# danieldugas/DeepMimic_mujoco

Hardware: AMD Instinct MI355X
Metric: env-steps/sec (whole node), 34-DoF humanoid, 4096 envs, at 1/2/4/8 MI355X (higher is better)
Workload: dtype f32

## Files before the change

### deepmimic_mujoco_amd/csrc/dm_abi.hip

```cpp
#include "../../include/deepmimic_hip.h"
#include "dm_device.h"
#include "dm_topology.h"

#include <math.h>
#include <stdio.h>
#include <string.h>

#include <string>
#include <vector>

#include "dm_kernels.hip"

struct DmEngine {
  DmConfig cfg;
  DmModel model;
  int N = 0;
  DmDev *dT = nullptr;
  float *dState = nullptr;
  float *dArScratch = nullptr;
  float *dClipRows[DM_MAX_CLIPS] = {nullptr};
  float *dClipReset[DM_MAX_CLIPS] = {nullptr};
  int clipL[DM_MAX_CLIPS] = {0};
  int clipFlags[DM_MAX_CLIPS] = {0};
  float *debug = nullptr;
// ... 85 lines not shown
    T.b_chainb[b] = cb;
  }
  for (int k = 0; k < DM_NV; k++) {
    int j = m.dof_jnt[k];
    T.d_body[k] = m.dof_body[k];
    T.d_act[k] = -1;
    T.d_limited[k] = (m.jnt_type[j] == DM_JNT_HINGE) ? m.jnt_limited[j] : 0;
    for (int i = 0; i < 3; i++) T.d_axis[k][i] = (float)m.jnt_axis[j][i];
    T.d_arm[k] = (float)m.dof_armature[k]; T.d_damp[k] = (float)m.dof_damping[k];
    T.d_invw[k] = (float)m.dof_invweight0[k];
    T.d_lo[k] = (float)m.jnt_range[j][0]; T.d_hi[k] = (float)m.jnt_range[j][1];
    int n = 0;
    for (int a = m.dof_parent[k]; a >= 0 && n < DMK_MAXANC; a = m.dof_parent[a]) T.d_anc[k][n++] = (uint8_t)a;
    T.d_nanc[k] = n;
    for (int d = 0; d < n; d++) T.d_ancabs[k][d] = T.d_anc[k][n - 1 - d];
    T.d_pbody[k] = m.body_parent[m.dof_body[k]];
  }
  for (int k = 0; k < DM_NV; k++) {
    for (int a = 0; a < T.d_nanc[k]; a++) T.d_desc[T.d_anc[k][a]] |= 1ull << k;
    T.nanc_pack[k >> 4] |= (uint64_t)T.d_nanc[k] << (4 * (k & 15));
    for (int a = 0; a < T.d_nanc[k]; a++) T.d_ancm[k] |= 1ull << T.d_anc[k][a];
    T.d_madr[k] = m.dof_Madr[k];
  }
  for (int a = 0; a < DM_NU; a++) {
    int k = m.act_dof[a];
    T.d_act[k] = a; T.d_gear[k] = (float)m.act_gear[a];
    T.d_clo[k] = (float)m.act_ctrlrange[a][0]; T.d_chi[k] = (float)m.act_ctrlrange[a][1];
  }
  for (int g = 0; g < DM_NGEOM; g++) {
    T.g_body[g] = m.geom_body[g]; T.g_type[g] = m.geom_type[g]; T.g_condim[g] = m.geom_condim[g];
    for (int i = 0; i < 3; i++) { T.g_pos[g][i] = (float)m.geom_pos[g][i]; T.g_size[g][i] = (float)m.geom_size[g][i]; }
    const double *q = m.geom_quat[g];
    double w = q[0], x = q[1], y = q[2], z = q[3];
    double M[9] = {w * w + x * x - y * y - z * z, 2 * (x * y - w * z), 2 * (x * z + w * y),
                   2 * (x * y + w * z), w * w - x * x + y * y - z * z, 2 * (y * z - w * x),
                   2 * (x * z - w * y), 2 * (y * z + w * x), w * w - x * x - y * y + z * z};
    for (int i = 0; i < 9; i++) T.g_mat[g][i] = (float)M[i];
    T.g_rbound[g] = (float)m.geom_rbound[g]; T.g_margin[g] = (float)m.geom_margin[g];
    T.g_mu[g] = (float)m.geom_friction[g][0];
  }
  for (int p = 0; p < DM_MAXPAIR; p++) { T.p_g1[p] = (int16_t)m.pair_geom1[p]; T.p_g2[p] = (int16_t)m.pair_geom2[p]; }
  for (int p = 0; p < m.npair; p++) {
    int g1 = m.pair_geom1[p], g2 = m.pair_geom2[p];
    DmPairDev &pr = T.pairs[p];
    pr.g1 = (int16_t)g1; pr.g2 = (int16_t)g2;
    pr.t1 = (int8_t)m.geom_type[g1]; pr.t2 = (int8_t)m.geom_type[g2];
    pr.margin = (float)fmax(m.geom_margin[g1], m.geom_margin[g2]);
    pr.rbsum = (float)((m.geom_type[g1] == DM_GEOM_PLANE ? 0.0 : m.geom_rbound[g1]) + m.geom_rbound[g2]);
    for (int i = 0; i < 3; i++) { pr.z1[i] = (float)m.geom_size[g1][i]; pr.z2[i] = (float)m.geom_size[g2][i]; }
  }
  int p = 0;
  for (int b = 0; b < DMK_MAXANC; b++)
    for (int a = 0; a <= b; a++) { T.tri_a[p] = (uint8_t)a; T.tri_b[p] = (uint8_t)b; p++; }
}

static int check_model(DmEngine *e, const DmModel &m) {
  if (m.nq != DM_NQ || m.nv != DM_NV || m.nu != DM_NU || m.nbody != DM_NBODY || m.ngeom != DM_NGEOM)
    return fail(e, DM_EINVAL, "model dimensions do not match the compiled-in humanoid3d dimensions");
  if (m.integrator != DM_INT_RK4 && m.integrator != DM_INT_EULER) return fail(e, DM_EINVAL, "integrator must be RK4 or Euler");
  if (m.npair < 0 || m.npair > DM_MAXPAIR) return fail(e, DM_EINVAL, "npair out of range");
  for (int b = 1; b < DM_NBODY; b++) {
    if (m.body_quat[b][0] != 1.0) return fail(e, DM_EINVAL, "kernels assume identity body quaternions");
    if (m.body_dofnum[b] != 1 && m.body_dofnum[b] != 3 && m.body_dofnum[b] != 6)
      return fail(e, DM_EINVAL, "kernels assume 1- or 3-hinge bodies under a free root");
    if (m.body_depth[b] < 1 || m.body_depth[b] > 4) return fail(e, DM_EINVAL, "tree depth > 4");
  }
  for (int j = 0; j < DM_NJNT; j++)
    for (int i = 0; i < 3; i++)
      if (m.jnt_pos[j][i] != 0.0) return fail(e, DM_EINVAL, "kernels assume joint anchors at the body origin");
  if (m.jnt_type[0] != DM_JNT_FREE || m.jnt_body[0] != 1) return fail(e, DM_EINVAL, "joint 0 must be the free root");
  for (int k = 0; k < DM_NV; k++)
    if (m.dof_parent[k] != topo::PARENT[k] || m.dof_Madr[k] != topo::MADR[k])
      return fail(e, DM_EINVAL, "dof tree differs from the compiled-in topology (regenerate csrc/dm_topology.h)");
  for (int b = 0; b < DM_NBODY; b++)
    if (m.body_parent[b] != topo::BPARENT[b])
      return fail(e, DM_EINVAL, "body tree differs from the compiled-in topology (regenerate csrc/dm_topology.h)");
  return DM_OK;
}

extern "C" int dm_create(const DmModel *model, const DmConfig *cfg, DmHandle *out) {
  if (!model || !cfg || !out || cfg->num_envs < 1) return DM_EINVAL;
  int ndev = 0;
  if (hipGetDeviceCount(&ndev) != hipSuccess || ndev <= 0) return DM_ENODEV;
  DmEngine *e = new DmEngine();
  e->cfg = *cfg;
  e->model = *model;
  e->N = cfg->num_envs;
  if (const char *w = getenv("DM_WAVES")) e->waves = atoi(w);
  int rc = check_model(e, *model);
  if (rc != DM_OK) { fprintf(stderr, "dm_create: %s\n", e->err.c_str()); delete e; return rc; }
  if (hipSetDevice(cfg->device) != hipSuccess) { delete e; return DM_ENODEV; }
  DmDev T;
  build_tables(*model, T);
  if (hipMalloc(&e->dT, sizeof(DmDev)) != hipSuccess) { delete e; return DM_ENOMEM; }
  hipMemcpy(e->dT, &T, sizeof(DmDev), hipMemcpyHostToDevice);
  size_t sb = (size_t)e->N * DMK_STATE_STRIDE * sizeof(float);
  if (hipMalloc(&e->dState, sb) != hipSuccess) { hipFree(e->dT); delete e; return DM_ENOMEM; }
  std::vector<float> init((size_t)e->N * DMK_STATE_STRIDE, 0.f);
  for (int i = 0; i < e->N; i++)
    for (int k = 0; k < DM_NQ; k++) init[(size_t)i * DMK_STATE_STRIDE + DMS_QPOS + k] = (float)model->qpos0[k];
  hipMemcpy(e->dState, init.data(), sb, hipMemcpyHostToDevice);
  if (hipMalloc(&e->dArScratch, (size_t)e->N * DMK_MAXROW * DMK_MAXROW * sizeof(float)) != hipSuccess) {
    hipFree(e->dState); hipFree(e->dT); delete e; return DM_ENOMEM;
  }
  if (hipMalloc(&e->dOrder, e->N * sizeof(int32_t)) != hipSuccess || hipMalloc(&e->dCost, e->N * sizeof(int32_t)) != hipSuccess) {
    hipFree(e->dArScratch); hipFree(e->dState); hipFree(e->dT); delete e; return DM_ENOMEM;
// ... 352 lines not shown
```

### deepmimic_mujoco_amd/csrc/dm_device.h

```cpp
#pragma once

#include <hip/hip_runtime.h>
#include <stdint.h>

#include "../../include/dm_model.h"

#define DMK_NQ DM_NQ
#define DMK_NV DM_NV
#define DMK_NU DM_NU
#define DMK_NB DM_NBODY
#define DMK_NG DM_NGEOM
#define DMK_MAXCON DM_MAXCON
#define DMK_MAXROW DM_MAXROW
#define DMK_LANEROW 64
#define DMK_REGROW 32
#define DMK_MSTRIDE 35
#define DMK_MAXANC 12
#define DMK_STATE_STRIDE 144
#define DMK_CLIP_ROW 80

struct DmPairDev {
  int16_t g1, g2;
  int8_t t1, t2, pad0, pad1;
  float margin, rbsum;
  float z1[3], z2[3];
};

struct DmDev {
  float timestep, tolerance, pgs_scale, gravity[3];
  float K, B;
  float solimp[5];
  float total_mass_inv;
  float qpos0[36];
  int32_t iterations, npair;
  int32_t torso_body, rfoot_geom, lfoot_geom, floor_geom;
  int32_t ee_geom[4];
  int32_t b_parent[16], b_depth[16], b_dofadr[16], b_dofnum[16];
  float b_pos[16][3], b_ipos[16][3], b_inertia[16][6], b_mass[16], b_invw[16];
  uint32_t b_subtree[16];
  uint64_t b_chain[16];
  uint32_t b_chainb[16];
  int32_t d_body[DM_NV], d_nanc[DM_NV], d_act[DM_NV], d_limited[DM_NV];
  float d_axis[DM_NV][3];
  float d_arm[DM_NV], d_damp[DM_NV], d_invw[DM_NV], d_lo[DM_NV], d_hi[DM_NV];
  float d_gear[DM_NV], d_clo[DM_NV], d_chi[DM_NV];
  uint8_t d_anc[DM_NV][DMK_MAXANC];
  uint8_t d_ancabs[DM_NV][DMK_MAXANC + 4];
  uint64_t d_desc[DM_NV];
  int32_t d_pbody[DM_NV];
  uint64_t nanc_pack[3];
  uint64_t d_ancm[DM_NV];
  int32_t d_madr[DM_NV];
  int32_t g_body[16], g_type[16], g_condim[16];
  float g_pos[16][3], g_mat[16][9], g_size[16][3], g_rbound[16], g_margin[16], g_mu[16];
  int16_t p_g1[DM_MAXPAIR], p_g2[DM_MAXPAIR];
  DmPairDev pairs[DM_MAXPAIR];
  uint8_t tri_a[80], tri_b[80];
};

struct EnvLds {
  float qpos[36], qvel[36], warm[36], ctrl[28];
  float qacc_smooth[36], qacc[36];
  float cs[36][2];
  float xpos[DMK_NB][3], xquat[DMK_NB][4], xmat[DMK_NB][9], xipos[DMK_NB][3];
  float xaxis[DMK_NV][3];
  float gpos[DMK_NG][3], gmat[DMK_NG][9];
  float com[4];
  float cinert[DMK_NB][10];
  float cdof[DMK_NV][8];
  float cvel[DMK_NB][6];
  float M[DM_NM + 2];
  float dinv[36], dsqrtinv[36];
  float rk[5][36], rkq[4];
  float c_dist[DMK_MAXCON], c_pos[DMK_MAXCON][3], c_frame[DMK_MAXCON][9];
  int32_t c_g1[DMK_MAXCON], c_g2[DMK_MAXCON];
#ifdef DM_PROFILE
  unsigned long long prof_t, prof_t0; unsigned prof[16], prof_stage[4];
#endif
  int32_t info[8];
  int16_t rowinfo[DMK_MAXROW];
  union {
    struct {
      float crb[DMK_NB][10];
      float qloc[DMK_NB][8];
      union {
        struct { float cdofdot[DMK_NV][6]; float cacc[DMK_NB][6]; };
        alignas(16) float mbuf[DMK_NV][8];
      };
      float cfrc[DMK_NB][6], cfrcsub[DMK_NB][6];
    } v;
    struct {
      float tr[20][DM_NV + 1];
    } fin;
    struct {
      float poly[2][16][3];
      float cand[8][8];
      int32_t ncand;
    } bb;
  } u;
};

#define DMS_QPOS 0
#define DMS_QVEL 35
#define DMS_WARM 69
#define DMS_CTRL 103
#define DMS_IDX 131
#define DMS_EPLEN 132
#define DMS_EPREW 133
#define DMS_CLIP 134
#define DMS_RCNT 135
#define DMS_F8R 136
// ... 39 lines not shown
```

### deepmimic_mujoco_amd/csrc/dm_kernels.hip

```cpp
#include "../../include/deepmimic_hip.h"
#include "dm_device.h"
#include "dm_rng.h"
#include "dm_topology.h"

#include <math.h>

#include <type_traits>

#define SYNC()                                              \
  do {                                                      \
    __builtin_amdgcn_fence(__ATOMIC_RELEASE, "wavefront");  \
    __builtin_amdgcn_wave_barrier();                        \
    __builtin_amdgcn_fence(__ATOMIC_ACQUIRE, "wavefront");  \
  } while (0)
#define DMK_ENVS_PER_BLOCK 1
#ifndef DMK_WAVES_PER_SIMD
#define DMK_WAVES_PER_SIMD 2
#endif
#ifdef DM_PROFILE
#define PROF_DECL do { if ((threadIdx.x & 63) == 0) { for (int _i = 0; _i < 16; _i++) g_S.prof[_i] = 0; for (int _i = 0; _i < 4; _i++) g_S.prof_stage[_i] = 0; g_S.prof_t = g_S.prof_t0 = __builtin_amdgcn_s_memtime(); } } while (0)
#define PROF_STAGE(i) do { if ((threadIdx.x & 63) == 0 && (i) < 4) g_S.prof_stage[i] = (unsigned)(__builtin_amdgcn_s_memtime() - g_S.prof_t0); } while (0)
#define PROF(i) do { if ((threadIdx.x & 63) == 0) { unsigned long long _t = __builtin_amdgcn_s_memtime(); g_S.prof[i] += (unsigned)(_t - g_S.prof_t); g_S.prof_t = _t; } } while (0)
#if DM_PROFILE == 2
#define PROF2(i) PROF(i)
#else
#define PROF2(i) do {} while (0)
#endif
#else
#define PROF2(i) do {} while (0)
#define PROF_STAGE(i) do {} while (0)
#define PROF_DECL do {} while (0)
#define PROF(i) do {} while (0)
#endif
typedef __attribute__((address_space(3))) const float *lds_cfloat_p;
typedef float lds_f2v __attribute__((ext_vector_type(2)));
typedef float lds_f4v __attribute__((ext_vector_type(4)));
typedef float mfma_f16v __attribute__((ext_vector_type(16)));
#ifndef DMK_MFMA_MIN_ROWS
#define DMK_MFMA_MIN_ROWS 8
#endif
typedef const __attribute__((address_space(1))) DmDev GDev;
typedef const __attribute__((address_space(1))) DmPairDev GPair;
#define MINVALF 1e-15f
#define MAXVALF 1e10f

namespace {

template <int I, int N>
struct StaticFor {
  template <class F>
  static __device__ __forceinline__ void run(F &&f) {
    if constexpr (I < N) {
      if (f(std::integral_constant<int, I>{})) StaticFor<I + 1, N>::run(f);
    }
  }
};

__device__ __forceinline__ float rl(float v, int lane) {
  return __int_as_float(__builtin_amdgcn_readlane(__float_as_int(v), lane));
}
template <unsigned long long MASK>
__device__ __forceinline__ float lane_sel(float a, float b) {
  float out;
  asm("v_cndmask_b32_e64 %0, %1, %2, %3" : "=v"(out) : "v"(b), "v"(a), "s"(MASK));
  return out;
}
template <unsigned long long MASK>
__device__ __forceinline__ int lane_sel_i(int a, int b) {
  int out;
  asm("v_cndmask_b32_e64 %0, %1, %2, %3" : "=v"(out) : "v"(b), "v"(a), "s"(MASK));
  return out;
}
template <int N>
__device__ __forceinline__ void sgpr_batch(float (&a)[topo::FS_SLOTS]) {
  static_assert(N >= 1 && N <= 8 && topo::FS_SLOTS == 8, "one asm statement per batch size");
  if constexpr (N == 1) asm("" : "+s"(a[0]));
  if constexpr (N == 2) asm("" : "+s"(a[0]), "+s"(a[1]));
  if constexpr (N == 3) asm("" : "+s"(a[0]), "+s"(a[1]), "+s"(a[2]));
  if constexpr (N == 4) asm("" : "+s"(a[0]), "+s"(a[1]), "+s"(a[2]), "+s"(a[3]));
  if constexpr (N == 5) asm("" : "+s"(a[0]), "+s"(a[1]), "+s"(a[2]), "+s"(a[3]), "+s"(a[4]));
  if constexpr (N == 6) asm("" : "+s"(a[0]), "+s"(a[1]), "+s"(a[2]), "+s"(a[3]), "+s"(a[4]), "+s"(a[5]));
  if constexpr (N == 7) asm("" : "+s"(a[0]), "+s"(a[1]), "+s"(a[2]), "+s"(a[3]), "+s"(a[4]), "+s"(a[5]), "+s"(a[6]));
  if constexpr (N == 8) asm("" : "+s"(a[0]), "+s"(a[1]), "+s"(a[2]), "+s"(a[3]), "+s"(a[4]), "+s"(a[5]), "+s"(a[6]), "+s"(a[7]));
}
__device__ __forceinline__ void factor_columns(float (&C)[DMK_NV]) {
  float d[topo::FS_SLOTS], m[topo::FS_SLOTS], rk[DMK_NV], Cs[DMK_NV];
  StaticFor<0, topo::FS_NOPS>::run([&](auto nc) {
    constexpr topo::FactorOp o = topo::FACTOR_SCHED[decltype(nc)::value];
    if constexpr (o.op == topo::FS_DIAG) d[o.slot] = rl(C[o.k], o.k);
    if constexpr (o.op == topo::FS_RCP) rk[o.k] = __builtin_amdgcn_rcpf(d[o.slot]);
    if constexpr (o.op == topo::FS_SCALE) Cs[o.k] = C[o.k] * rk[o.k];
    if constexpr (o.op == topo::FS_BCAST) m[o.slot] = rl(Cs[o.k], o.i);
    if constexpr (o.op == topo::FS_FMA) C[o.i] = fmaf(-m[o.slot], C[o.k], C[o.i]);
    if constexpr (o.op == topo::FS_FENCE) sgpr_batch<o.slot>(m);
    if constexpr (o.op == topo::FS_DFENCE) sgpr_batch<o.slot>(d);
// ... 375 lines not shown
  S.u.bb.ncand = cnt;
}

__device__ __noinline__ float impedance_pow(float x, float mid, float power) {
  return (x <= mid) ? powf(x, power) / powf(mid, power - 1) : 1 - powf(1 - x, power) / powf(1 - mid, power - 1);
}
__device__ __forceinline__ float impedance(const float *solimp, float pos, float margin) {
  float dmin = solimp[0], dmax = solimp[1], width = solimp[2], mid = solimp[3], power = solimp[4];
  if (dmin == dmax || width <= MINVALF) return 0.5f * (dmin + dmax);
  float x = fabsf(pos - margin) / width;
  if (x >= 1) return dmax;
  if (x <= 0) return dmin;
  float y;
  if (power == 1) y = x;
  else if (power == 2) y = (x <= mid) ? x * x / mid : 1 - (1 - x) * (1 - x) / (1 - mid);
  else y = impedance_pow(x, mid, power);
  return dmin + y * (dmax - dmin);
}

}

__shared__ EnvLds g_S;

#define bp (T.b_parent[lb])
#define bdofadr (T.b_dofadr[lb])
#define bdofnum (T.b_dofnum[lb])
#define bpos (T.b_pos[lb])
#define bipos (T.b_ipos[lb])
#define binert (T.b_inertia[lb])
#define bsub (T.b_subtree[lb])
#define baxis(j) (T.d_axis[(bdofadr + (j)) < DMK_NV ? (bdofadr + (j)) : 0])
#define dbody (T.d_body[lk])
#define dnanc (T.d_nanc[lk])
#define dact (T.d_act[lk])
#define dlimited (T.d_limited[lk])
#define darm (T.d_arm[lk])
#define ddamp (T.d_damp[lk])
#define dlo (T.d_lo[lk])
#define dhi (T.d_hi[lk])
#define dgear (T.d_gear[lk])
#define dclo (T.d_clo[lk])
#define dchi (T.d_chi[lk])
#define gbody (T.g_body[lg])
#define gposl (T.g_pos[lg])
#define gmatl (T.g_mat[lg])

template <bool DAMP2 = false>
__device__ __forceinline__ float fwd_smooth(GDev &T, const int lane, const float rhs = 0.f) {
  EnvLds &S = g_S;
  const int lb = lane < DMK_NB ? lane : 0;
  const int lk = lane < DMK_NV ? lane : 0;
  const int lg = lane < DMK_NG ? lane : 0;
  const bool isbody = lane >= 1 && lane < DMK_NB, isdof = lane < DMK_NV;
  const float bmass = (lane < DMK_NB) ? T.b_mass[lb] : 0.f;
  const int b_dofadr = T.b_dofadr[lb], b_dofnum = T.b_dofnum[lb];
  const uint32_t b_chain4 = T.b_chainb[lb];
  const unsigned b_sub = T.b_subtree[lb];
  const int d_body = T.d_body[lk], d_nanc = T.d_nanc[lk], d_pbody = T.d_pbody[lk];
  const float mtot_inv = T.total_mass_inv;

  if constexpr (!DAMP2) {
  {
    float q[4] = {S.qpos[3], S.qpos[4], S.qpos[5], S.qpos[6]};
    quat_normalize(q);
    SYNC();
    if (lane < 4) S.qpos[3 + lane] = (lane == 0) ? q[0] : (lane == 1) ? q[1] : (lane == 2) ? q[2] : q[3];
    if (lane >= 6 && lane < DMK_NV) {
      float sn, cs;
      sincosf(0.5f * S.qpos[lane + 1], &sn, &cs);
      S.cs[lane][0] = cs; S.cs[lane][1] = sn;
    }
    SYNC();
  }
  PROF2(12);
  if (isbody) {
    float q[4] = {1.f, 0.f, 0.f, 0.f};
    if (lb == 1) {
      for (int i = 0; i < 4; i++) q[i] = S.qpos[3 + i];
    } else {
      {
        const int k = b_dofadr;
        const float al[3] = {T.d_axis[k][0], T.d_axis[k][1], T.d_axis[k][2]};
        S.xaxis[k][0] = al[0]; S.xaxis[k][1] = al[1]; S.xaxis[k][2] = al[2];
        const float c = S.cs[k][0], sn = S.cs[k][1];
        q[0] = c; q[1] = al[0] * sn; q[2] = al[1] * sn; q[3] = al[2] * sn;
      }
#pragma unroll
      for (int j = 1; j < 3; j++) {
        if (j < b_dofnum) {
          const int k = b_dofadr + j;
          const float al[3] = {T.d_axis[k][0], T.d_axis[k][1], T.d_axis[k][2]};
          float ax[3], ql[4], qn[4];
          quat_rot(ax, q, al);
          S.xaxis[k][0] = ax[0]; S.xaxis[k][1] = ax[1]; S.xaxis[k][2] = ax[2];
          const float c = S.cs[k][0], sn = S.cs[k][1];
          ql[0] = c; ql[1] = al[0] * sn; ql[2] = al[1] * sn; ql[3] = al[2] * sn;
          quat_mul(qn, q, ql);
          q[0] = qn[0]; q[1] = qn[1]; q[2] = qn[2]; q[3] = qn[3];
        }
      }
    }
    for (int i = 0; i < 4; i++) S.u.v.qloc[lb][i] = q[i];
    for (int i = 0; i < 3; i++) S.u.v.qloc[lb][4 + i] = (lb == 1) ? S.qpos[i] : T.b_pos[lb][i];
  }
  SYNC();
  if (isbody) {
    float q[4], pos[3];
    for (int i = 0; i < 4; i++) q[i] = S.u.v.qloc[1][i];
    for (int i = 0; i < 3; i++) pos[i] = S.u.v.qloc[1][4 + i];
#pragma unroll
    for (int c = 1; c < 4; c++) {
      const int cb = (b_chain4 >> (8 * c)) & 0xFF;
      if (cb != 0) {
        float ql[4], pl[3], t[3], qn[4];
        for (int i = 0; i < 4; i++) ql[i] = S.u.v.qloc[cb][i];
        for (int i = 0; i < 3; i++) pl[i] = S.u.v.qloc[cb][4 + i];
        quat_rot(t, q, pl);
        pos[0] += t[0]; pos[1] += t[1]; pos[2] += t[2];
        quat_mul(qn, q, ql);
        q[0] = qn[0]; q[1] = qn[1]; q[2] = qn[2]; q[3] = qn[3];
      }
    }
    quat_normalize(q);
    float m9[9], tv[3];
    quat2mat(m9, q);
    const float ip[3] = {T.b_ipos[lb][0], T.b_ipos[lb][1], T.b_ipos[lb][2]};
    mat_vec(tv, m9, ip);
    for (int i = 0; i < 3; i++) { S.xpos[lb][i] = pos[i]; S.xipos[lb][i] = pos[i] + tv[i]; }
    for (int i = 0; i < 4; i++) S.xquat[lb][i] = q[i];
    for (int i = 0; i < 9; i++) S.xmat[lb][i] = m9[i];
  }
  SYNC();
  PROF2(13);
  float com[3];
  {
    float ax[3] = {0.f, 0.f, 0.f};
    if (lane >= 6 && isdof) {
      const float pq[4] = {S.xquat[d_pbody][0], S.xquat[d_pbody][1], S.xquat[d_pbody][2], S.xquat[d_pbody][3]};
      const float al[3] = {S.xaxis[lk][0], S.xaxis[lk][1], S.xaxis[lk][2]};
      quat_rot(ax, pq, al);
    } else if (lane >= 3 && lane < 6) {
      ax[0] = S.xmat[1][lane - 3]; ax[1] = S.xmat[1][3 + lane - 3]; ax[2] = S.xmat[1][6 + lane - 3];
    }
    if (lane < DMK_NG) {
      const int gb = T.g_body[lg];
      float bm[9], tv[3], gl[3] = {T.g_pos[lg][0], T.g_pos[lg][1], T.g_pos[lg][2]}, gm[9];
      for (int i = 0; i < 9; i++) { bm[i] = S.xmat[gb][i]; gm[i] = T.g_mat[lg][i]; }
      mat_vec(tv, bm, gl);
      for (int i = 0; i < 3; i++) S.gpos[lg][i] = S.xpos[gb][i] + tv[i];
      for (int i = 0; i < 3; i++)
        for (int j = 0; j < 3; j++)
          S.gmat[lg][3 * i + j] = bm[3 * i] * gm[j] + bm[3 * i + 1] * gm[3 + j] + bm[3 * i + 2] * gm[6 + j];
    }
    const float xi[3] = {S.xipos[lb][0], S.xipos[lb][1], S.xipos[lb][2]};
    for (int i = 0; i < 3; i++) com[i] = wave_sum(bmass * xi[i]) * mtot_inv;
    if (lane == 0) { S.com[0] = com[0]; S.com[1] = com[1]; S.com[2] = com[2]; }
    SYNC();
    if (isdof) {
      float cd[6] = {0, 0, 0, 0, 0, 0};
      if (lane < 3) {
        cd[3 + lane] = 1.f;
      } else {
        const float off[3] = {com[0] - S.xpos[d_body][0], com[1] - S.xpos[d_body][1], com[2] - S.xpos[d_body][2]};
        cd[0] = ax[0]; cd[1] = ax[1]; cd[2] = ax[2];
        cross3(cd + 3, ax, off);
        S.xaxis[lk][0] = ax[0]; S.xaxis[lk][1] = ax[1]; S.xaxis[lk][2] = ax[2];
      }
      for (int i = 0; i < 6; i++) S.cdof[lk][i] = cd[i];
      S.cdof[lk][6] = 0; S.cdof[lk][7] = 0;
    }
  }
  PROF2(14);
  if (isbody) {
    float R[9], Tm[9], W[6], bi[6];
    for (int i = 0; i < 9; i++) R[i] = S.xmat[lb][i];
    for (int i = 0; i < 6; i++) bi[i] = T.b_inertia[lb][i];
    const float Ib[9] = {bi[0], bi[3], bi[4], bi[3], bi[1], bi[5], bi[4], bi[5], bi[2]};
    for (int i = 0; i < 3; i++)
      for (int j = 0; j < 3; j++) Tm[3 * i + j] = R[3 * i] * Ib[j] + R[3 * i + 1] * Ib[3 + j] + R[3 * i + 2] * Ib[6 + j];
    W[0] = Tm[0] * R[0] + Tm[1] * R[1] + Tm[2] * R[2];
    W[1] = Tm[3] * R[3] + Tm[4] * R[4] + Tm[5] * R[5];
    W[2] = Tm[6] * R[6] + Tm[7] * R[7] + Tm[8] * R[8];
    W[3] = Tm[0] * R[3] + Tm[1] * R[4] + Tm[2] * R[5];
    W[4] = Tm[0] * R[6] + Tm[1] * R[7] + Tm[2] * R[8];
    W[5] = Tm[3] * R[6] + Tm[4] * R[7] + Tm[5] * R[8];
    const float o[3] = {S.xipos[lb][0] - com[0], S.xipos[lb][1] - com[1], S.xipos[lb][2] - com[2]};
    const float oo = dot3(o, o);
    float *ci = S.cinert[lb];
    ci[0] = W[0] + bmass * (oo - o[0] * o[0]);
    ci[1] = W[1] + bmass * (oo - o[1] * o[1]);
    ci[2] = W[2] + bmass * (oo - o[2] * o[2]);
    ci[3] = W[3] - bmass * o[0] * o[1];
    ci[4] = W[4] - bmass * o[0] * o[2];
    ci[5] = W[5] - bmass * o[1] * o[2];
    ci[6] = bmass * o[0]; ci[7] = bmass * o[1]; ci[8] = bmass * o[2];
    ci[9] = bmass;
  }
  SYNC();
  PROF(1);
  }
  {
    float acc[10];
    for (int i = 0; i < 10; i++) acc[i] = 0;
    StaticFor<1, DMK_NB>::run([&](auto cc) {
      constexpr int c = decltype(cc)::value;
      const float w = lane_sel<topo::body_ancself_mask(c)>(1.f, 0.f);
#pragma unroll
      for (int i = 0; i < 10; i++) acc[i] = fmaf(w, g_S.cinert[c][i], acc[i]);
      return true;
    });
    if (isbody)
      for (int i = 0; i < 10; i++) S.u.v.crb[lb][i] = acc[i];
  }
  SYNC();
  float C[DMK_NV];
  {
    float cd[6] = {0, 0, 0, 0, 0, 0};
    if (isdof) {
      float buf[6], I[10];
      for (int i = 0; i < 10; i++) I[i] = S.u.v.crb[d_body][i];
      for (int i = 0; i < 6; i++) cd[i] = S.cdof[lk][i];
      mul_inert_vec(buf, I, cd);
      for (int i = 0; i < 6; i++) S.u.v.mbuf[lk][i] = buf[i];
    }
    SYNC();
    const float armv = isdof ? (DAMP2 ? fmaf(T.timestep, T.d_damp[lk], T.d_arm[lk]) : T.d_arm[lk]) : 0.f;
    float dots[DMK_NV];
    {
      const float *bufp = &S.u.v.mbuf[lane & 31][lane >> 5];
      mfma_f16v acc;
#pragma unroll
      for (int v = 0; v < 16; v++) acc[v] = 0.f;
#pragma unroll
      for (int p = 0; p < 3; p++) {
        const auto sw = __builtin_amdgcn_permlane32_swap(__float_as_uint(cd[2 * p]), __float_as_uint(cd[2 * p + 1]), false, false);
        acc = __builtin_amdgcn_mfma_f32_32x32x2f32(bufp[2 * p], __uint_as_float(sw[0]), acc, 0, 0, 0);
      }
#pragma unroll
      for (int v = 0; v < 16; v++) {
        const auto sw = __builtin_amdgcn_permlane32_swap(__float_as_uint(acc[v]), __float_as_uint(acc[v]), false, false);
        dots[(v / 4) * 8 + (v % 4)] = acc[v];
        dots[(v / 4) * 8 + (v % 4) + 4] = __uint_as_float(sw[1]);
      }
#pragma unroll
      for (int k = 32; k < DMK_NV; k++) {
        float d = 0;
#pragma unroll
        for (int i = 0; i < 6; i++) d = fmaf(cd[i], S.u.v.mbuf[k][i], d);
        dots[k] = d;
      }
    }
    StaticFor<0, DMK_NV>::run([&](auto kc) {
      constexpr int k = decltype(kc)::value;
      const float off = lane_sel<topo::anc_mask(k)>(dots[k], 0.f);
      C[k] = lane_sel<(1ull << k)>(dots[k] + armv, off);
      return true;
    });
  }
  PROF(2);
  factor_columns(C);
  const int d_nanc_s = isdof ? d_nanc : 0;
  {
    StaticFor<0, DMK_NV>::run([&](auto kc) {
      constexpr int k = decltype(kc)::value;
      const int real = topo::MADR[k] + topo::NANC[k] - d_nanc_s;
      const int idx = lane_sel_i<(topo::anc_mask(k) | (1ull << k))>(real, DM_NM + 1);
      g_S.M[idx] = C[k];
      return true;
    });
  }
  SYNC();
  float dv = 0.f;
  const int mrow = T.d_madr[lk] + d_nanc;
  const uint64_t ancm = T.d_ancm[lk];
  if (isdof) {
    const float Md = S.M[T.d_madr[lk]];
    dv = 1.0f / Md;
    S.dinv[lk] = dv;
    S.dsqrtinv[lk] = 1.0f / sqrtf(Md);
  }
  SYNC();
  PROF(3);
  float xs = 0;
  if constexpr (DAMP2) {
    xs = isdof ? rhs : 0.f;
  } else {
  if (isbody) {
    float w[6] = {0, 0, 0, 0, 0, 0};
    const int nd = (lb == 1) ? 6 : b_dofnum;
    for (int j = 0; j < 6; j++)
      if (j < nd) {
        const int k = b_dofadr + j;
        const float qv = S.qvel[k];
        for (int i = 0; i < 6; i++) w[i] += S.cdof[k][i] * qv;
      }
    for (int i = 0; i < 6; i++) S.u.v.cacc[lb][i] = w[i];
  }
  SYNC();
  if (isbody) {
    float cv[6] = {0, 0, 0, 0, 0, 0}, u[6] = {0, 0, 0, 0, 0, 0};
#pragma unroll
    for (int c = 0; c < 3; c++) {
      const int cb = (b_chain4 >> (8 * c)) & 0xFF;
      if (cb != 0 && cb != lb)
        for (int i = 0; i < 6; i++) cv[i] += S.u.v.cacc[cb][i];
    }
    if (lb == 1) {
      for (int k = 0; k < 3; k++) {
        const float qv = S.qvel[k];
        for (int i = 0; i < 6; i++) cv[i] += S.cdof[k][i] * qv;
      }
      float dd[3][6];
#pragma unroll
      for (int k = 3; k < 6; k++) {
        float cd[6];
        for (int i = 0; i < 6; i++) cd[i] = S.cdof[k][i];
        cross_motion(dd[k - 3], cv, cd);
      }
#pragma unroll
      for (int k = 3; k < 6; k++) {
        const float qv = S.qvel[k];
        for (int i = 0; i < 6; i++) { u[i] += dd[k - 3][i] * qv; cv[i] += S.cdof[k][i] * qv; }
      }
    } else {
#pragma unroll
      for (int j = 0; j < 3; j++) {
        if (j < b_dofnum) {
          const int k = b_dofadr + j;
          float cd[6], dd[6];
          const float qv = S.qvel[k];
          for (int i = 0; i < 6; i++) cd[i] = S.cdof[k][i];
          cross_motion(dd, cv, cd);
          for (int i = 0; i < 6; i++) { u[i] += dd[i] * qv; cv[i] += cd[i] * qv; }
        }
      }
    }
    for (int i = 0; i < 6; i++) { S.cvel[lb][i] = cv[i]; S.u.v.cfrcsub[lb][i] = u[i]; }
  }
  SYNC();
  PROF2(15);
  if (isbody) {
    float ca[6] = {0, 0, 0, -T.gravity[0], -T.gravity[1], -T.gravity[2]}, cv[6], I[10], f0[6], t0[6], t1[6];
#pragma unroll
    for (int c = 0; c < 4; c++) {
      const int cb = (b_chain4 >> (8 * c)) & 0xFF;
      if (cb != 0)
        for (int i = 0; i < 6; i++) ca[i] += S.u.v.cfrcsub[cb][i];
    }
    for (int i = 0; i < 6; i++) cv[i] = S.cvel[lb][i];
    for (int i = 0; i < 10; i++) I[i] = S.cinert[lb][i];
    mul_inert_vec(f0, I, ca);
    mul_inert_vec(t0, I, cv);
    cross_force(t1, cv, t0);
    for (int i = 0; i < 6; i++) S.u.v.cfrc[lb][i] = f0[i] + t1[i];
  }
  SYNC();
  {
    float acc[6] = {0, 0, 0, 0, 0, 0};
    StaticFor<1, DMK_NB>::run([&](auto cc) {
      constexpr int c = decltype(cc)::value;
      const float w = lane_sel<topo::body_ancself_mask(c)>(1.f, 0.f);
#pragma unroll
      for (int i = 0; i < 6; i++) acc[i] = fmaf(w, g_S.u.v.cfrc[c][i], acc[i]);
      return true;
    });
    if (isbody)
      for (int i = 0; i < 6; i++) S.u.v.cacc[lb][i] = acc[i];
  }
  SYNC();
  PROF2(10);
  if (isdof) {
    float bias = 0;
    for (int i = 0; i < 6; i++) bias += S.cdof[lk][i] * S.u.v.cacc[d_body][i];
    float act = 0;
    const int da = T.d_act[lk];
    if (da >= 0) act = T.d_gear[lk] * clampf(S.ctrl[da], T.d_clo[lk], T.d_chi[lk]);
    xs = -T.d_damp[lk] * S.qvel[lk] - bias + act;
  }
  }
  xs = solve_LT(xs, dv, -d_nanc_s, g_S.M);
  xs = solve_L(xs, dv, isdof ? mrow : DMK_MAXANC, g_S.M);
  xs *= dv;
  if constexpr (!DAMP2) {
    if (isdof) S.qacc_smooth[lk] = xs;
  }
  SYNC();
  PROF(4);
  return xs;
}

__device__ __noinline__ float euler_damped_solve(GDev &T, const int lane, const float rhs) {
  return fwd_smooth<true>(T, lane, rhs);
}

__device__ __forceinline__ int fwd_collide(GDev &T, const int lane) {
  EnvLds &S = g_S;
  int ncon = 0, overflow = 0;
  const int lb = lane < DMK_NB ? lane : 0;
  const int lk = lane < DMK_NV ? lane : 0;
  const int lg = lane < DMK_NG ? lane : 0;
  const int bdep = (lane < DMK_NB) ? T.b_depth[lb] : -1;
  const float bmass = (lane < DMK_NB) ? T.b_mass[lb] : 0.f;
  const float mtot_inv = T.total_mass_inv;
  (void)lg; (void)bdep; (void)bmass; (void)mtot_inv; (void)lb; (void)lk;
    int base = 0;
    overflow = 0;
    for (int round = 0; round < 2; round++) {
      const int p = round * 64 + lane;
      Cand c;
      c.valid = 0;
      c.t[0] = c.t[1] = c.t[2] = 0;
#pragma unroll
      for (int s = 0; s < 4; s++) {
        c.d[s] = 0;
#pragma unroll
        for (int i = 0; i < 3; i++) { c.p[s][i] = 0; c.n[s][i] = 0; }
      }
      int g1 = 0, g2 = 0;
      bool isbb = false;
      float margin = 0;
      bool act = false;
      int t1 = 0, t2 = 0;
      float x1[3], x2[3], z1[3], z2[3];
      if (p < T.npair) {
        GPair &pr = T.pairs[p];
        g1 = pr.g1; g2 = pr.g2; t1 = pr.t1; t2 = pr.t2;
        margin = pr.margin;
        for (int i = 0; i < 3; i++) { x1[i] = S.gpos[g1][i]; x2[i] = S.gpos[g2][i]; z1[i] = pr.z1[i]; z2[i] = pr.z2[i]; }
        const float df[3] = {x2[0] - x1[0], x2[1] - x1[1], x2[2] - x1[2]};
        if (t1 == DM_GEOM_PLANE) {
// ... 150 lines not shown
              c.d[s] = S.u.bb.cand[s][0];
              for (int q = 0; q < 3; q++) { c.p[s][q] = S.u.bb.cand[s][1 + q]; c.n[s][q] = S.u.bb.cand[s][4 + q]; }
            }
        }
      }
      int cnt = __popc(c.valid);
      unsigned long long lt = lanemask_lt(lane);
      unsigned long long b0 = __ballot(cnt & 1), b1 = __ballot(cnt & 2), b2 = __ballot(cnt & 4);
      int off = __popcll(b0 & lt) + 2 * __popcll(b1 & lt) + 4 * __popcll(b2 & lt);
      int total = __popcll(b0) + 2 * __popcll(b1) + 4 * __popcll(b2);
      if (total == 0) continue;
      int w = base + off;
#pragma unroll
      for (int s = 0; s < 4; s++) {
        if ((c.valid >> s) & 1) {
          if (w < DMK_MAXCON) {
            float fr[9] = {c.n[s][0], c.n[s][1], c.n[s][2], c.t[0], c.t[1], c.t[2], 0, 0, 0};
            make_frame(fr);
            S.c_dist[w] = c.d[s];
            for (int q = 0; q < 3; q++) S.c_pos[w][q] = c.p[s][q];
            for (int q = 0; q < 9; q++) S.c_frame[w][q] = fr[q];
            S.c_g1[w] = g1; S.c_g2[w] = g2;
          }
          w++;
        }
      }
      base += total;
    }
    if (base > DMK_MAXCON) { overflow |= 1; base = DMK_MAXCON; }
    ncon = base;
    SYNC();

    PROF(5);
  return ncon | (overflow << 8);
}

template <bool MF, bool PF = true>
__device__ __forceinline__ void build_row(GDev &T, EnvLds &S, const int r, const int nefc, const float (&com)[3],
                                          float (&J)[DMK_NV], float &R, float &Dd, float &aref, float &bb, float &jw) {
      float rpos = 0, rmargin = 0, rdiag = 1, mu = 0;
      int rtype = -1;
      float wl[3] = {0, 0, 0}, wa[3] = {0, 0, 0};
      unsigned long long cm1 = 0, cm2 = 0;
      int ldof = -1;
      float lsign = 0;
      if (r < nefc) {
        int info = S.rowinfo[r];
        if (info < 0) {
          int v = -info - 1;
          ldof = v >> 1;
          lsign = (v & 1) ? -1.f : 1.f;
          rtype = 0;
          float q = S.qpos[ldof + 1];
          rpos = (v & 1) ? (T.d_hi[ldof] - q) : (q - T.d_lo[ldof]);
          rmargin = 0;
          rdiag = T.d_invw[ldof];
        } else {
          int ci = (info >> 3) & 0x3F, e = info & 7;
          int g1 = S.c_g1[ci], g2 = S.c_g2[ci];
          int b1 = T.g_body[g1], b2 = T.g_body[g2];
          int cd1 = T.g_condim[g1], cd2 = T.g_condim[g2];
          int dim = cd1 > cd2 ? cd1 : cd2;
          mu = fmaxf(T.g_mu[g1], T.g_mu[g2]);
          float fr[9];
          for (int i = 0; i < 9; i++) fr[i] = S.c_frame[ci][i];
          float tran = T.b_invw[b1] + T.b_invw[b2];
          if (dim < 3) {
            rtype = 1;
            wl[0] = fr[0]; wl[1] = fr[1]; wl[2] = fr[2];
            rdiag = tran;
          } else {
            rtype = 2;
            const bool second = (e >> 1) != 0;
            const float tx = second ? fr[6] : fr[3], ty = second ? fr[7] : fr[4], tz = second ? fr[8] : fr[5];
            float sg = (e & 1) ? -mu : mu;
            wl[0] = fr[0] + sg * tx; wl[1] = fr[1] + sg * ty; wl[2] = fr[2] + sg * tz;
            rdiag = tran + mu * mu * tran;
          }
          float off[3] = {S.c_pos[ci][0] - com[0], S.c_pos[ci][1] - com[1], S.c_pos[ci][2] - com[2]};
          cross3(wa, off, wl);
          cm1 = T.b_chain[b1]; cm2 = T.b_chain[b2];
          rpos = S.c_dist[ci];
          rmargin = fmaxf(T.g_margin[g1], T.g_margin[g2]);
        }
      }
      float vel = 0, jqs = 0;
      jw = 0;
      float vals[32];
      if (MF) {
        const float wv[6] = {wa[0], wa[1], wa[2], wl[0], wl[1], wl[2]};
        const int lane_ = (int)(threadIdx.x & 63);
        const float *cdp = &S.cdof[lane_ & 31][lane_ >> 5];
        mfma_f16v acc;
#pragma unroll
        for (int v = 0; v < 16; v++) acc[v] = 0.f;
#pragma unroll
        for (int p = 0; p < 3; p++) {
          const auto sw = __builtin_amdgcn_permlane32_swap(__float_as_uint(wv[2 * p]), __float_as_uint(wv[2 * p + 1]), false, false);
          acc = __builtin_amdgcn_mfma_f32_32x32x2f32(cdp[2 * p], __uint_as_float(sw[0]), acc, 0, 0, 0);
        }
#pragma unroll
        for (int v = 0; v < 16; v++) {
          const auto sw = __builtin_amdgcn_permlane32_swap(__float_as_uint(acc[v]), __float_as_uint(acc[v]), false, false);
          vals[(v / 4) * 8 + (v % 4)] = acc[v];
          vals[(v / 4) * 8 + (v % 4) + 4] = __uint_as_float(sw[1]);
        }
      }
#pragma unroll
      for (int k = 0; k < DMK_NV; k++) {
        float val;
        if (MF && k < 32) {
          val = vals[k];
        } else {
          const float4 ca = *reinterpret_cast<const float4 *>(&S.cdof[k][0]);
          const float2 cb = *reinterpret_cast<const float2 *>(&S.cdof[k][4]);
          val = ca.x * wa[0] + ca.y * wa[1] + ca.z * wa[2] + ca.w * wl[0] + cb.x * wl[1] + cb.y * wl[2];
        }
        float sg = (float)((int)((cm2 >> k) & 1ull) - (int)((cm1 >> k) & 1ull));
        float j = (k == ldof) ? lsign : sg * val;
        J[k] = j;
        vel += j * S.qvel[k];
        jqs += j * S.qacc_smooth[k];
        jw += j * S.warm[k];
      }
      R = 1; Dd = 0; aref = 0; bb = 0;
      if (r < nefc) {
        float sol[5] = {T.solimp[0], T.solimp[1], T.solimp[2], T.solimp[3], T.solimp[4]};
        float imp = impedance(sol, rpos, rmargin);
        R = fmaxf(MINVALF, (1 - imp) * rdiag / imp);
        if (rtype == 2) R = 2 * mu * mu * R;
        aref = -T.B * vel - T.K * imp * (rpos - rmargin);
        bb = jqs - aref;
        Dd = 1.0f / R;
      }
      {
        if constexpr (PF) {
// ... 826 lines not shown
```

Baseline: 14.21 million.

## Pack per-lane model constants into 16-byte records for vector loads

Adds per-lane body, dof, geom, contact-row and limit-row records to the device model, built once on the host. The forward kernel and the constraint-row builder then fetch each lane's constants with a few 128-bit global loads instead of many scattered scalar loads across separate arrays. This trades a larger constant table and some register pressure from loads hoisted early for fewer global load instructions.

```diff
diff --git a/deepmimic_mujoco_amd/csrc/dm_abi.hip b/deepmimic_mujoco_amd/csrc/dm_abi.hip
--- a/deepmimic_mujoco_amd/csrc/dm_abi.hip
+++ b/deepmimic_mujoco_amd/csrc/dm_abi.hip
@@ -161,6 +161,7 @@
   int p = 0;
   for (int b = 0; b < DMK_MAXANC; b++)
     for (int a = 0; a <= b; a++) { T.tri_a[p] = (uint8_t)a; T.tri_b[p] = (uint8_t)b; p++; }
+  dm_build_lane_records(T);
 }
 
 static int check_model(DmEngine *e, const DmModel &m) {
diff --git a/deepmimic_mujoco_amd/csrc/dm_device.h b/deepmimic_mujoco_amd/csrc/dm_device.h
--- a/deepmimic_mujoco_amd/csrc/dm_device.h
+++ b/deepmimic_mujoco_amd/csrc/dm_device.h
@@ -4,6 +4,7 @@
 #include <stdint.h>
 
 #include "../../include/dm_model.h"
+#include "dm_tables.h"
 
 #define DMK_NQ DM_NQ
 #define DMK_NV DM_NV
@@ -15,48 +16,8 @@
 #define DMK_LANEROW 64
 #define DMK_REGROW 32
 #define DMK_MSTRIDE 35
-#define DMK_MAXANC 12
 #define DMK_STATE_STRIDE 144
 #define DMK_CLIP_ROW 80
-
-struct DmPairDev {
-  int16_t g1, g2;
-  int8_t t1, t2, pad0, pad1;
-  float margin, rbsum;
-  float z1[3], z2[3];
-};
-
-struct DmDev {
-  float timestep, tolerance, pgs_scale, gravity[3];
-  float K, B;
-  float solimp[5];
-  float total_mass_inv;
-  float qpos0[36];
-  int32_t iterations, npair;
-  int32_t torso_body, rfoot_geom, lfoot_geom, floor_geom;
-  int32_t ee_geom[4];
-  int32_t b_parent[16], b_depth[16], b_dofadr[16], b_dofnum[16];
-  float b_pos[16][3], b_ipos[16][3], b_inertia[16][6], b_mass[16], b_invw[16];
-  uint32_t b_subtree[16];
-  uint64_t b_chain[16];
-  uint32_t b_chainb[16];
-  int32_t d_body[DM_NV], d_nanc[DM_NV], d_act[DM_NV], d_limited[DM_NV];
-  float d_axis[DM_NV][3];
-  float d_arm[DM_NV], d_damp[DM_NV], d_invw[DM_NV], d_lo[DM_NV], d_hi[DM_NV];
-  float d_gear[DM_NV], d_clo[DM_NV], d_chi[DM_NV];
-  uint8_t d_anc[DM_NV][DMK_MAXANC];
-  uint8_t d_ancabs[DM_NV][DMK_MAXANC + 4];
-  uint64_t d_desc[DM_NV];
-  int32_t d_pbody[DM_NV];
-  uint64_t nanc_pack[3];
-  uint64_t d_ancm[DM_NV];
-  int32_t d_madr[DM_NV];
-  int32_t g_body[16], g_type[16], g_condim[16];
-  float g_pos[16][3], g_mat[16][9], g_size[16][3], g_rbound[16], g_margin[16], g_mu[16];
-  int16_t p_g1[DM_MAXPAIR], p_g2[DM_MAXPAIR];
-  DmPairDev pairs[DM_MAXPAIR];
-  uint8_t tri_a[80], tri_b[80];
-};
 
 struct EnvLds {
   float qpos[36], qvel[36], warm[36], ctrl[28];
diff --git a/deepmimic_mujoco_amd/csrc/dm_kernels.hip b/deepmimic_mujoco_amd/csrc/dm_kernels.hip
--- a/deepmimic_mujoco_amd/csrc/dm_kernels.hip
+++ b/deepmimic_mujoco_amd/csrc/dm_kernels.hip
@@ -41,6 +41,13 @@
 #endif
 typedef const __attribute__((address_space(1))) DmDev GDev;
 typedef const __attribute__((address_space(1))) DmPairDev GPair;
+typedef uint32_t rec_u4 __attribute__((ext_vector_type(4)));
+typedef const __attribute__((address_space(1))) rec_u4 GRec4;
+typedef const __attribute__((address_space(1))) char GByte;
+#define REC4(T, role, idx, c)                                                                                    \
+  (*(GRec4 *)((GByte *)&(T) + ((unsigned)(offsetof(DmDev, rec) + offsetof(DmLaneRec, role) + 16 * (c)) +         \
+                               (unsigned)(idx) * (unsigned)sizeof(((DmLaneRec *)nullptr)->role[0]))))
+#define RECF(x) __uint_as_float(x)
 #define MINVALF 1e-15f
 #define MAXVALF 1e10f
 
@@ -522,14 +529,14 @@
   const int lk = lane < DMK_NV ? lane : 0;
   const int lg = lane < DMK_NG ? lane : 0;
   const bool isbody = lane >= 1 && lane < DMK_NB, isdof = lane < DMK_NV;
-  const float bmass = (lane < DMK_NB) ? T.b_mass[lb] : 0.f;
-  const int b_dofadr = T.b_dofadr[lb], b_dofnum = T.b_dofnum[lb];
-  const uint32_t b_chain4 = T.b_chainb[lb];
-  const unsigned b_sub = T.b_subtree[lb];
-  const int d_body = T.d_body[lk], d_nanc = T.d_nanc[lk], d_pbody = T.d_pbody[lk];
+  const rec_u4 rd0 = REC4(T, dof, lane, 0);
+  const int d_body = (int)rd0.x, d_nanc = (int)rd0.y, d_pbody = (int)rd0.z;
   const float mtot_inv = T.total_mass_inv;
 
   if constexpr (!DAMP2) {
+  const rec_u4 rb0 = REC4(T, body, lane, 0), rb1 = REC4(T, body, lane, 1), rb2 = REC4(T, body, lane, 2),
+               rb3 = REC4(T, body, lane, 3), rb4 = REC4(T, body, lane, 4);
+  const float bmass = (lane < DMK_NB) ? RECF(rb1.w) : 0.f;
   {
     float q[4] = {S.qpos[3], S.qpos[4], S.qpos[5], S.qpos[6]};
     quat_normalize(q);
@@ -549,17 +556,17 @@
       for (int i = 0; i < 4; i++) q[i] = S.qpos[3 + i];
     } else {
       {
-        const int k = b_dofadr;
-        const float al[3] = {T.d_axis[k][0], T.d_axis[k][1], T.d_axis[k][2]};
+        const int k = (int)rb0.x;
+        const float al[3] = {RECF(rb2.x), RECF(rb2.y), RECF(rb2.z)};
         S.xaxis[k][0] = al[0]; S.xaxis[k][1] = al[1]; S.xaxis[k][2] = al[2];
         const float c = S.cs[k][0], sn = S.cs[k][1];
         q[0] = c; q[1] = al[0] * sn; q[2] = al[1] * sn; q[3] = al[2] * sn;
       }
 #pragma unroll
       for (int j = 1; j < 3; j++) {
-        if (j < b_dofnum) {
-          const int k = b_dofadr + j;
-          const float al[3] = {T.d_axis[k][0], T.d_axis[k][1], T.d_axis[k][2]};
+        if (j < (int)rb0.y) {
+          const int k = (int)rb0.x + j;
+          const float al[3] = {RECF(j == 1 ? rb2.w : rb3.z), RECF(j == 1 ? rb3.x : rb3.w), RECF(j == 1 ? rb3.y : rb4.x)};
           float ax[3], ql[4], qn[4];
           quat_rot(ax, q, al);
           S.xaxis[k][0] = ax[0]; S.xaxis[k][1] = ax[1]; S.xaxis[k][2] = ax[2];
@@ -571,9 +578,12 @@
       }
     }
     for (int i = 0; i < 4; i++) S.u.v.qloc[lb][i] = q[i];
-    for (int i = 0; i < 3; i++) S.u.v.qloc[lb][4 + i] = (lb == 1) ? S.qpos[i] : T.b_pos[lb][i];
+    for (int i = 0; i < 3; i++) S.u.v.qloc[lb][4 + i] = (lb == 1) ? S.qpos[i] : RECF(rb1[i]);
   }
   SYNC();
+  const rec_u4 rb5 = REC4(T, body, lane, 5), rb6 = REC4(T, body, lane, 6);
+  const rec_u4 rg0 = REC4(T, geom, lane, 0), rg1 = REC4(T, geom, lane, 1), rg2 = REC4(T, geom, lane, 2), rg3 = REC4(T, geom, lane, 3);
+  const uint32_t b_chain4 = rb0.z;
   if (isbody) {
     float q[4], pos[3];
     for (int i = 0; i < 4; i++) q[i] = S.u.v.qloc[1][i];
@@ -594,7 +604,7 @@
     quat_normalize(q);
     float m9[9], tv[3];
     quat2mat(m9, q);
-    const float ip[3] = {T.b_ipos[lb][0], T.b_ipos[lb][1], T.b_ipos[lb][2]};
+    const float ip[3] = {RECF(rb4.y), RECF(rb4.z), RECF(rb4.w)};
     mat_vec(tv, m9, ip);
     for (int i = 0; i < 3; i++) { S.xpos[lb][i] = pos[i]; S.xipos[lb][i] = pos[i] + tv[i]; }
     for (int i = 0; i < 4; i++) S.xquat[lb][i] = q[i];
@@ -613,9 +623,11 @@
       ax[0] = S.xmat[1][lane - 3]; ax[1] = S.xmat[1][3 + lane - 3]; ax[2] = S.xmat[1][6 + lane - 3];
     }
     if (lane < DMK_NG) {
-      const int gb = T.g_body[lg];
-      float bm[9], tv[3], gl[3] = {T.g_pos[lg][0], T.g_pos[lg][1], T.g_pos[lg][2]}, gm[9];
-      for (int i = 0; i < 9; i++) { bm[i] = S.xmat[gb][i]; gm[i] = T.g_mat[lg][i]; }
+      const int gb = (int)rg0.w;
+      const float gl[3] = {RECF(rg0.x), RECF(rg0.y), RECF(rg0.z)};
+      const float gm[9] = {RECF(rg1.x), RECF(rg1.y), RECF(rg1.z), RECF(rg1.w), RECF(rg2.x), RECF(rg2.y), RECF(rg2.z), RECF(rg2.w), RECF(rg3.x)};
+      float bm[9], tv[3];
+      for (int i = 0; i < 9; i++) bm[i] = S.xmat[gb][i];
       mat_vec(tv, bm, gl);
       for (int i = 0; i < 3; i++) S.gpos[lg][i] = S.xpos[gb][i] + tv[i];
       for (int i = 0; i < 3; i++)
@@ -644,7 +656,7 @@
   if (isbody) {
     float R[9], Tm[9], W[6], bi[6];
     for (int i = 0; i < 9; i++) R[i] = S.xmat[lb][i];
-    for (int i = 0; i < 6; i++) bi[i] = T.b_inertia[lb][i];
+    bi[0] = RECF(rb5.x); bi[1] = RECF(rb5.y); bi[2] = RECF(rb5.z); bi[3] = RECF(rb5.w); bi[4] = RECF(rb6.x); bi[5] = RECF(rb6.y);
     const float Ib[9] = {bi[0], bi[3], bi[4], bi[3], bi[1], bi[5], bi[4], bi[5], bi[2]};
     for (int i = 0; i < 3; i++)
       for (int j = 0; j < 3; j++) Tm[3 * i + j] = R[3 * i] * Ib[j] + R[3 * i + 1] * Ib[3 + j] + R[3 * i + 2] * Ib[6 + j];
@@ -694,7 +706,7 @@
       for (int i = 0; i < 6; i++) S.u.v.mbuf[lk][i] = buf[i];
     }
     SYNC();
-    const float armv = isdof ? (DAMP2 ? fmaf(T.timestep, T.d_damp[lk], T.d_arm[lk]) : T.d_arm[lk]) : 0.f;
+    const float armv = isdof ? (DAMP2 ? fmaf(T.timestep, RECF(REC4(T, dof, lane, 1).z), T.d_arm[lk]) : T.d_arm[lk]) : 0.f;
     float dots[DMK_NV];
     {
       const float *bufp = &S.u.v.mbuf[lane & 31][lane >> 5];
@@ -729,6 +741,7 @@
   }
   PROF(2);
   factor_columns(C);
+  const rec_u4 rv0 = REC4(T, body, lane, 0), rd1 = REC4(T, dof, lane, 1), rd2 = REC4(T, dof, lane, 2);
   const int d_nanc_s = isdof ? d_nanc : 0;
   {
     StaticFor<0, DMK_NV>::run([&](auto kc) {
@@ -741,10 +754,9 @@
   }
   SYNC();
   float dv = 0.f;
-  const int mrow = T.d_madr[lk] + d_nanc;
-  const uint64_t ancm = T.d_ancm[lk];
+  const int mrow = (int)rd1.x + d_nanc;
   if (isdof) {
-    const float Md = S.M[T.d_madr[lk]];
+    const float Md = S.M[(int)rd1.x];
     dv = 1.0f / Md;
     S.dinv[lk] = dv;
     S.dsqrtinv[lk] = 1.0f / sqrtf(Md);
@@ -755,6 +767,8 @@
   if constexpr (DAMP2) {
     xs = isdof ? rhs : 0.f;
   } else {
+  const int b_dofadr = (int)rv0.x, b_dofnum = (int)rv0.y;
+  const uint32_t b_chain4 = rv0.z;
   if (isbody) {
     float w[6] = {0, 0, 0, 0, 0, 0};
     const int nd = (lb == 1) ? 6 : b_dofnum;
@@ -843,9 +857,9 @@
     float bias = 0;
     for (int i = 0; i < 6; i++) bias += S.cdof[lk][i] * S.u.v.cacc[d_body][i];
     float act = 0;
-    const int da = T.d_act[lk];
-    if (da >= 0) act = T.d_gear[lk] * clampf(S.ctrl[da], T.d_clo[lk], T.d_chi[lk]);
-    xs = -T.d_damp[lk] * S.qvel[lk] - bias + act;
+    const int da = (int)rd1.y;
+    if (da >= 0) act = RECF(rd1.w) * clampf(S.ctrl[da], RECF(rd2.x), RECF(rd2.y));
+    xs = -RECF(rd1.z) * S.qvel[lk] - bias + act;
   }
   }
   xs = solve_LT(xs, dv, -d_nanc_s, g_S.M);
@@ -1102,19 +1116,38 @@
           lsign = (v & 1) ? -1.f : 1.f;
           rtype = 0;
           float q = S.qpos[ldof + 1];
-          rpos = (v & 1) ? (T.d_hi[ldof] - q) : (q - T.d_lo[ldof]);
+          float lo, hi;
+          if constexpr (PF) {
+            lo = T.rec.lrow[ldof].lo; hi = T.rec.lrow[ldof].hi; rdiag = T.rec.lrow[ldof].invw;
+          } else {
+            lo = T.d_lo[ldof]; hi = T.d_hi[ldof]; rdiag = T.d_invw[ldof];
+          }
+          rpos = (v & 1) ? (hi - q) : (q - lo);
           rmargin = 0;
-          rdiag = T.d_invw[ldof];
         } else {
           int ci = (info >> 3) & 0x3F, e = info & 7;
           int g1 = S.c_g1[ci], g2 = S.c_g2[ci];
-          int b1 = T.g_body[g1], b2 = T.g_body[g2];
-          int cd1 = T.g_condim[g1], cd2 = T.g_condim[g2];
+          int cd1, cd2;
+          float mu1, mu2, iw1, iw2, mg1, mg2;
+          if constexpr (PF) {
+            const rec_u4 ra0 = REC4(T, crow, g1, 0), ra1 = REC4(T, crow, g1, 1), rb0 = REC4(T, crow, g2, 0), rb1 = REC4(T, crow, g2, 1);
+            cd1 = (int)ra0.x; cd2 = (int)rb0.x;
+            mu1 = RECF(ra0.y); mu2 = RECF(rb0.y); mg1 = RECF(ra0.z); mg2 = RECF(rb0.z);
+            iw1 = RECF(ra0.w); iw2 = RECF(rb0.w);
+            cm1 = (unsigned long long)ra1.x | ((unsigned long long)ra1.y << 32);
+            cm2 = (unsigned long long)rb1.x | ((unsigned long long)rb1.y << 32);
+          } else {
+            const int b1 = T.g_body[g1], b2 = T.g_body[g2];
+            cd1 = T.g_condim[g1]; cd2 = T.g_condim[g2];
+            mu1 = T.g_mu[g1]; mu2 = T.g_mu[g2]; mg1 = T.g_margin[g1]; mg2 = T.g_margin[g2];
+            iw1 = T.b_invw[b1]; iw2 = T.b_invw[b2];
+            cm1 = T.b_chain[b1]; cm2 = T.b_chain[b2];
+          }
           int dim = cd1 > cd2 ? cd1 : cd2;
-          mu = fmaxf(T.g_mu[g1], T.g_mu[g2]);
+          mu = fmaxf(mu1, mu2);
           float fr[9];
           for (int i = 0; i < 9; i++) fr[i] = S.c_frame[ci][i];
-          float tran = T.b_invw[b1] + T.b_invw[b2];
+          float tran = iw1 + iw2;
           if (dim < 3) {
             rtype = 1;
             wl[0] = fr[0]; wl[1] = fr[1]; wl[2] = fr[2];
@@ -1129,9 +1162,8 @@
           }
           float off[3] = {S.c_pos[ci][0] - com[0], S.c_pos[ci][1] - com[1], S.c_pos[ci][2] - com[2]};
           cross3(wa, off, wl);
-          cm1 = T.b_chain[b1]; cm2 = T.b_chain[b2];
           rpos = S.c_dist[ci];
-          rmargin = fmaxf(T.g_margin[g1], T.g_margin[g2]);
+          rmargin = fmaxf(mg1, mg2);
         }
       }
       float vel = 0, jqs = 0;
diff --git a/deepmimic_mujoco_amd/csrc/dm_tables.h b/deepmimic_mujoco_amd/csrc/dm_tables.h
--- /dev/null
+++ b/deepmimic_mujoco_amd/csrc/dm_tables.h
@@ -0,0 +1,119 @@
+#pragma once
+
+#include <stdint.h>
+#include <string.h>
+
+#include "../../include/dm_model.h"
+
+#define DMK_MAXANC 12
+#define DMK_REC_LANES 64
+
+struct DmPairDev {
+  int16_t g1, g2;
+  int8_t t1, t2, pad0, pad1;
+  float margin, rbsum;
+  float z1[3], z2[3];
+};
+
+struct alignas(16) DmBodyRec {
+  int32_t dofadr, dofnum; uint32_t chainb, subtree;
+  float pos[3], mass;
+  float axis[3][3];
+  float ipos[3];
+  float inertia[6]; uint32_t pad[2];
+};
+struct alignas(16) DmDofRec {
+  int32_t body, nanc, pbody; float arm;
+  int32_t madr, act; float damp, gear;
+  float clo, chi; uint64_t ancm;
+};
+struct alignas(16) DmGeomRec {
+  float pos[3]; int32_t body;
+  float mat[9]; uint32_t pad[3];
+};
+struct alignas(16) DmContactRowRec {
+  int32_t condim; float mu, margin, invw;
+  uint64_t chain; int32_t body; uint32_t pad;
+};
+struct alignas(16) DmLimitRowRec {
+  float lo, hi, invw; uint32_t pad;
+};
+static_assert(sizeof(DmBodyRec) == 112 && sizeof(DmDofRec) == 48 && sizeof(DmGeomRec) == 64 && sizeof(DmContactRowRec) == 32 &&
+              sizeof(DmLimitRowRec) == 16, "the kernels address the records by 16-byte chunk");
+struct alignas(16) DmLaneRec {
+  DmBodyRec body[DMK_REC_LANES];
+  DmDofRec dof[DMK_REC_LANES];
+  DmGeomRec geom[DMK_REC_LANES];
+  DmContactRowRec crow[DM_NGEOM];
+  DmLimitRowRec lrow[DM_NV];
+};
+
+struct DmDev {
+  float timestep, tolerance, pgs_scale, gravity[3];
+  float K, B;
+  float solimp[5];
+  float total_mass_inv;
+  float qpos0[36];
+  int32_t iterations, npair;
+  int32_t torso_body, rfoot_geom, lfoot_geom, floor_geom;
+  int32_t ee_geom[4];
+  int32_t b_parent[16], b_depth[16], b_dofadr[16], b_dofnum[16];
+  float b_pos[16][3], b_ipos[16][3], b_inertia[16][6], b_mass[16], b_invw[16];
+  uint32_t b_subtree[16];
+  uint64_t b_chain[16];
+  uint32_t b_chainb[16];
+  int32_t d_body[DM_NV], d_nanc[DM_NV], d_act[DM_NV], d_limited[DM_NV];
+  float d_axis[DM_NV][3];
+  float d_arm[DM_NV], d_damp[DM_NV], d_invw[DM_NV], d_lo[DM_NV], d_hi[DM_NV];
+  float d_gear[DM_NV], d_clo[DM_NV], d_chi[DM_NV];
+  uint8_t d_anc[DM_NV][DMK_MAXANC];
+  uint8_t d_ancabs[DM_NV][DMK_MAXANC + 4];
+  uint64_t d_desc[DM_NV];
+  int32_t d_pbody[DM_NV];
+  uint64_t nanc_pack[3];
+  uint64_t d_ancm[DM_NV];
+  int32_t d_madr[DM_NV];
+  int32_t g_body[16], g_type[16], g_condim[16];
+  float g_pos[16][3], g_mat[16][9], g_size[16][3], g_rbound[16], g_margin[16], g_mu[16];
+  int16_t p_g1[DM_MAXPAIR], p_g2[DM_MAXPAIR];
+  DmPairDev pairs[DM_MAXPAIR];
+  uint8_t tri_a[80], tri_b[80];
+  DmLaneRec rec;
+};
+
+static inline void dm_build_lane_records(DmDev &T) {
+  DmLaneRec &R = T.rec;
+  memset(&R, 0, sizeof(R));
+  for (int l = 0; l < DMK_REC_LANES; l++) {
+    const int b = l < DM_NBODY ? l : 0, k = l < DM_NV ? l : 0, g = l < DM_NGEOM ? l : 0;
+    DmBodyRec &rb = R.body[l];
+    for (int i = 0; i < 3; i++) { rb.pos[i] = T.b_pos[b][i]; rb.ipos[i] = T.b_ipos[b][i]; }
+    for (int i = 0; i < 6; i++) rb.inertia[i] = T.b_inertia[b][i];
+    rb.mass = T.b_mass[b];
+    rb.dofadr = T.b_dofadr[b]; rb.dofnum = T.b_dofnum[b];
+    rb.chainb = T.b_chainb[b]; rb.subtree = T.b_subtree[b];
+    for (int j = 0; j < 3; j++) {
+      const int d = T.b_dofadr[b] + j;
+      if (j < T.b_dofnum[b] && d >= 0 && d < DM_NV)
+        for (int i = 0; i < 3; i++) rb.axis[j][i] = T.d_axis[d][i];
+    }
+    DmDofRec &rd = R.dof[l];
+    rd.body = T.d_body[k]; rd.nanc = T.d_nanc[k]; rd.pbody = T.d_pbody[k]; rd.madr = T.d_madr[k];
+    rd.ancm = T.d_ancm[k]; rd.arm = T.d_arm[k]; rd.damp = T.d_damp[k];
+    rd.act = T.d_act[k]; rd.gear = T.d_gear[k]; rd.clo = T.d_clo[k]; rd.chi = T.d_chi[k];
+    DmGeomRec &rg = R.geom[l];
+    for (int i = 0; i < 3; i++) rg.pos[i] = T.g_pos[g][i];
+    for (int i = 0; i < 9; i++) rg.mat[i] = T.g_mat[g][i];
+    rg.body = T.g_body[g];
+  }
+  for (int g = 0; g < DM_NGEOM; g++) {
+    DmContactRowRec &rc = R.crow[g];
+    const int b = T.g_body[g];
+    rc.body = b; rc.condim = T.g_condim[g]; rc.mu = T.g_mu[g]; rc.margin = T.g_margin[g];
+    if (b >= 0 && b < DM_NBODY) { rc.chain = T.b_chain[b]; rc.invw = T.b_invw[b]; }
+  }
+  for (int k = 0; k < DM_NV; k++) {
+    DmLimitRowRec &rl = R.lrow[k];
+    rl.lo = T.d_lo[k]; rl.hi = T.d_hi[k]; rl.invw = T.d_invw[k];
+  }
+}
```

After: 14.61 million, median of 6. 1.03x the previous value.
